# heitorrapela/HalluciDet

Measured on AMD Instinct MI355X. Metric: images/sec train_hallucidet (640x512, batch 8/GPU), higher is better.
Workload: dtype f16; 1 GPU; train_hallucidet.py fasterrcnn LLVIP batch=8 fp16 on 1xMI355X (BASELINE configs[1]); U-Net resnet34 fwd+bwd, 3 frozen Faster R-CNN R50-FPN passes @300x300 (one batched evaluation of 24 images: trunk, RPN, RoI heads, NMS for all three; the RGB / IR passes' LOSS VALUES, which the reference computes and discards, are not evaluated), loss scaling, value clip 0.5, Adam; global_batch=8, image=1x512x640 IR + 3x512x640 RGB, batch_per_gpu=8, parallelism=dp1

## Files before the change

### hallucidet_amd/_abi.py

```python
import ctypes as C
import os

_HERE = os.path.dirname(os.path.abspath(__file__))
LIB_PATH = os.environ.get("HD_HIP_LIB") or os.path.join(_HERE, "lib", "libhallucidet_hip.so")

ABI_VERSION = 6

HD_ACT_NONE, HD_ACT_RELU, HD_ACT_SIGMOID = 0, 1, 2
HD_OUT_NHWC_F16, HD_OUT_NCHW_F32, HD_OUT_NHWC_F32 = 0, 1, 2

c_i32 = C.c_int32
c_i64 = C.c_int64
c_f = C.c_float
c_d = C.c_double
vp = C.c_void_p


class HipLibraryMissing(RuntimeError):
    pass


class HipCallError(RuntimeError):
    pass

# ... 5 lines not shown
        ("C1", c_i32), ("C2", c_i32), ("Ho", c_i32), ("Wo", c_i32), ("Cout", c_i32),
        ("KH", c_i32), ("KW", c_i32), ("stride", c_i32), ("pad", c_i32),
        ("up1", c_i32), ("in_dil", c_i32), ("act", c_i32), ("out_mode", c_i32),
        ("in_scale", vp), ("in_shift", vp), ("in_relu", c_i32), ("out_pool2", c_i32),
        ("bs_y", vp), ("bs_z", vp), ("bs_mean", vp), ("bs_invstd", vp), ("bs_gamma", vp), ("bs_beta", vp), ("bs_relu", c_i32), ("reserved1", c_i32),
        ("y2", vp),
    ]


class WprepDesc(C.Structure):
    _fields_ = [("w_oihw", C.c_void_p), ("w_fwd", C.c_void_p), ("w_dgrad", C.c_void_p)] + \
               [(n, C.c_int32) for n in ("Cout", "Cin", "KH", "KW", "Cin_pad", "Cout_pad")]


class WredDesc(C.Structure):
    _fields_ = [("slab", C.c_void_p), ("dw_oihw", C.c_void_p)] + \
               [(n, C.c_int32) for n in ("nsplit", "Cout_slab", "Cout", "KH", "KW", "Cin", "Cin_real", "accumulate")] + \
               [("scale", C.c_float)] + [(n, C.c_int32) for n in ("mode", "first_block", "reserved")]


class WgradArgs(C.Structure):
    _fields_ = [
        ("x", vp), ("x2", vp), ("dy", vp), ("slab", vp),
        ("N", c_i32), ("Hsrc", c_i32), ("Wsrc", c_i32), ("Hin", c_i32), ("Win", c_i32),
        ("C1", c_i32), ("C2", c_i32), ("Ho", c_i32), ("Wo", c_i32), ("Cout", c_i32),
        ("KH", c_i32), ("KW", c_i32), ("stride", c_i32), ("pad", c_i32), ("up1", c_i32),
        ("nsplit", c_i32),
        ("in_scale", vp), ("in_shift", vp), ("in_relu", c_i32), ("reserved0", c_i32),
        ("dw_oihw", vp), ("dw_scale", c_f), ("reserved1", c_i32),
    ]


class ThinDgradArgs(C.Structure):
    _fields_ = [("ga", vp), ("gb", vp), ("wda", vp), ("wdb", vp), ("mask", vp), ("dx", vp), ("stride_a", c_i64), ("stride_b", c_i64)] + \
               [(n, c_i32) for n in ("n", "hw", "C", "Ka", "Kb", "Ka_p", "Kb_p", "g_f16")]


PROTOTYPES = {
    "hd_abi_version": (C.c_int, []),
    "hd_last_error": (C.c_char_p, []),
    "hd_arch": (C.c_char_p, []),
    "hd_conv2d": (C.c_int, [C.POINTER(ConvArgs), vp]),
    "hd_conv2d_stats_rows": (C.c_int, [C.POINTER(ConvArgs)]),
    "hd_conv2d_pool2_ok": (C.c_int, [C.POINTER(ConvArgs)]),
    "hd_conv2d_bstat_ok": (C.c_int, [C.POINTER(ConvArgs)]),
    "hd_conv2d_route": (C.c_int, [C.POINTER(ConvArgs), C.POINTER(c_i32)]),
    "hd_conv7x7s2_dgrad_thin": (C.c_int, [vp, vp, vp, vp] + [C.c_int] * 5 + [vp]),
    "hd_conv_tune_override": (C.c_int, [C.c_int] * 4),
    "hd_conv_tune_w8": (C.c_int, [C.c_int, C.c_int]),
    "hd_conv_nominal_batch": (C.c_int, [C.c_int]),
    "hd_gemm_w8_mode": (C.c_int, [C.c_int]),
    "hd_thin_gemm_mode": (C.c_int, [C.c_int]),
    "hd_thin_gemm_on": (C.c_int, []),
    "hd_thin_dgrad_pair": (C.c_int, [C.POINTER(ThinDgradArgs), vp]),
    "hd_thin_dgrad_pair_multi": (C.c_int, [C.POINTER(ThinDgradArgs), C.c_int, vp]),
    "hd_wgrad_w8_blocks": (C.c_int, [C.POINTER(WgradArgs)]),
    "hd_wgrad_route": (C.c_int, [C.POINTER(WgradArgs), C.POINTER(c_i32)]),
    "hd_wgrad": (C.c_int, [C.POINTER(WgradArgs), vp]),
    "hd_wgrad_multi": (C.c_int, [C.POINTER(WgradArgs), C.c_int, vp]),
    "hd_wgrad_direct_ok": (C.c_int, [C.POINTER(WgradArgs)]),
    "hd_conv2d_wgrad": (C.c_int, [C.POINTER(ConvArgs), C.POINTER(WgradArgs), vp]),
    "hd_conv2d_multi": (C.c_int, [C.POINTER(ConvArgs), C.c_int, vp]),
    "hd_wgrad_tune_override": (C.c_int, [C.c_int]),
    "hd_wgrad_reduce": (C.c_int, [vp, vp] + [C.c_int] * 7 + [c_f, C.c_int, vp]),
    "hd_wgrad_reduce_plan": (C.c_int, [vp, C.c_int]),
    "hd_wgrad_reduce_multi": (C.c_int, [vp, C.c_int, C.c_int, vp]),
    "hd_weight_prep": (C.c_int, [vp, vp, vp, vp] + [C.c_int] * 6 + [vp]),
    "hd_weight_prep_multi": (C.c_int, [vp, C.c_int, C.c_int, vp]),
    "hd_colsum": (C.c_int, [vp, C.c_int, C.c_int, vp, vp, vp]),
    "hd_rowsum": (C.c_int, [vp, C.c_int, C.c_int, vp, C.c_int, vp]),
    "hd_bn_finalize": (C.c_int, [vp, C.c_int, C.c_int, c_d, vp, vp, vp, vp, c_f, c_f, vp, vp, vp, vp, vp]),
    "hd_bn_eval_scale_shift": (C.c_int, [vp, vp, vp, vp, c_f, C.c_int, vp, vp, vp]),
    "hd_bn_apply": (C.c_int, [vp, vp, vp, vp, vp, c_i64, C.c_int, C.c_int, vp]),
    "hd_bn_bwd_reduce": (C.c_int, [vp] * 8 + [C.c_int, c_i64, C.c_int, C.c_int, vp]),
    "hd_bn_bwd_apply": (C.c_int, [vp] * 8 + [C.c_int] + [vp] * 5 + [c_f, C.c_int, c_i64, C.c_int, C.c_int, vp]),
    "hd_maxpool3x3s2": (C.c_int, [vp, vp] + [C.c_int] * 6 + [vp]),
    "hd_maxpool3x3s2_bwd": (C.c_int, [vp, vp, vp] + [C.c_int] * 6 + [vp]),
    "hd_maxpool3x3s2_idx": (C.c_int, [vp, vp, vp] + [C.c_int] * 6 + [vp]),
    "hd_maxpool3x3s2_bwd_idx": (C.c_int, [vp, vp, vp] + [C.c_int] * 6 + [vp]),
    "hd_maxpool3x3s2_bwd_idx_add": (C.c_int, [vp, vp, vp, vp] + [C.c_int] * 6 + [vp]),
    "hd_concat_up_bwd": (C.c_int, [vp, vp, vp] + [C.c_int] * 5 + [vp]),
    "hd_subsample2": (C.c_int, [vp, vp] + [C.c_int] * 6 + [vp]),
    "hd_subsample2_bwd": (C.c_int, [vp, vp] + [C.c_int] * 7 + [vp]),
    "hd_nchw_to_nhwc_resize": (C.c_int, [vp, vp] + [C.c_int] * 7 + [vp]),
    "hd_nchw_to_nhwc_resize_strided": (C.c_int, [vp, c_i64, c_i64, vp] + [C.c_int] * 7 + [vp]),
    "hd_nchw_to_nhwc_resize_bwd": (C.c_int, [vp, vp] + [C.c_int] * 7 + [c_f, vp]),
    "hd_image_resample": (C.c_int, [vp, c_i64, c_i64, vp] + [C.c_int] * 7 + [vp, vp, vp, C.c_int] * 2 + [vp, vp, vp, vp, vp]),
    "hd_image_resample_bwd": (C.c_int, [vp, vp] + [C.c_int] * 7 + [vp, vp, vp, C.c_int] * 2 + [vp, c_f, vp]),
    "hd_resample_taps_check": (C.c_int, [vp, vp, vp] + [C.c_int] * 3 + [vp, vp, vp, C.c_int, vp]),
    "hd_nhwc_to_nchw": (C.c_int, [vp, vp] + [C.c_int] * 5 + [vp]),
    "hd_upsample_add": (C.c_int, [vp, vp, vp] + [C.c_int] * 6 + [vp]),
    "hd_upsample_add_bwd": (C.c_int, [vp, vp] + [C.c_int] * 7 + [vp]),
    "hd_upsample2_bwd": (C.c_int, [vp, vp] + [C.c_int] * 7 + [vp]),
    "hd_add_f16": (C.c_int, [vp, vp, vp, c_i64, vp]),
    "hd_slice_channels": (C.c_int, [vp, vp, c_i64, C.c_int, C.c_int, C.c_int, C.c_int, vp]),
    "hd_sigmoid_bwd_nchw_to_nhwc": (C.c_int, [vp, vp, vp] + [C.c_int] * 5 + [c_f, vp]),
    "hd_relu_bwd": (C.c_int, [vp, vp, vp, c_i64, vp]),
    "hd_f32_to_f16": (C.c_int, [vp, vp, c_i64, c_f, vp]),
    "hd_f16_to_f32": (C.c_int, [vp, vp, c_i64, c_f, vp]),
    "hd_pad_cast_f32_f16": (C.c_int, [vp, vp, C.c_int64, C.c_int, C.c_int, C.c_int64, C.c_int64, vp]),
    "hd_pad_cast_f32_f16_multi": (C.c_int, [vp, vp, vp, vp, vp, vp, vp, C.c_int, vp]),
    "hd_channel_sum_f16": (C.c_int, [vp, c_i64, C.c_int, vp, C.c_int, vp]),
    "hd_scale_store": (C.c_int, [vp, vp, C.c_int, c_f, C.c_int, vp]),
    "hd_nms_sorted_batched": (C.c_int, [vp, vp, C.c_int, C.c_int, c_f, vp, vp, vp]),
    "hd_nms_sorted_batched_topk": (C.c_int, [vp, vp, C.c_int, C.c_int, c_f, vp, vp, C.c_int, vp]),
    "hd_roi_align": (C.c_int, [vp, vp, vp] + [C.c_int] * 7 + [c_f, C.c_int, vp]),
# ... 107 lines not shown
```

### hallucidet_amd/csrc/conv3x3_small.hip

```cpp
#include "hd_common.h"
#include "conv_params.h"

namespace {

typedef float f32x4_t __attribute__((ext_vector_type(4)));

constexpr int TH = 8, TW = 32;
constexpr int PH = TH + 2, PW = TW + 2;

__device__ __forceinline__ float row16_sum(float v) {
  v += __builtin_bit_cast(float, __builtin_amdgcn_update_dpp(0, __builtin_bit_cast(int, v), 0xB1, 0xF, 0xF, true));
  v += __builtin_bit_cast(float, __builtin_amdgcn_update_dpp(0, __builtin_bit_cast(int, v), 0x4E, 0xF, 0xF, true));
  v += __builtin_bit_cast(float, __builtin_amdgcn_update_dpp(0, __builtin_bit_cast(int, v), 0x141, 0xF, 0xF, true));
  v += __builtin_bit_cast(float, __builtin_amdgcn_update_dpp(0, __builtin_bit_cast(int, v), 0x140, 0xF, 0xF, true));
  return v;
}

template <int CIN, int COUT>
__global__ __launch_bounds__(256) void conv3x3_small_kernel(ConvP p) {
  constexpr int KTOT = 9 * CIN;
  constexpr int KSTEPS = (KTOT + 31) / 32;
  constexpr int KPAD = KSTEPS * 32;
  constexpr int MT = COUT / 16;
  constexpr int TPS = 32 / CIN;
  constexpr int PATCH_HALVES = PH * PW * CIN > 16 * TH * TW * 2 ? PH * PW * CIN : 16 * TH * TW * 2;
  __shared__ __attribute__((aligned(16))) f16 s_patch[PATCH_HALVES];
  __shared__ __attribute__((aligned(16))) f16 s_w[COUT * KPAD];
  __shared__ float s_red[4][COUT][2];

  const int tid = threadIdx.x, lane = tid & 63, wave = tid >> 6;
  const int tiles_x = (p.Wo + TW - 1) / TW, tiles_y = (p.Ho + TH - 1) / TH;
  const int tiles_total = p.N * tiles_x * tiles_y;

  for (int e = tid; e < COUT * KPAD / 8; e += 256) {
    const int co = e / (KPAD / 8), k8 = (e - co * (KPAD / 8)) * 8;
    f16x8 v = {0, 0, 0, 0, 0, 0, 0, 0};
    if (k8 < KTOT && co < p.Cout) v = *reinterpret_cast<const f16x8*>(p.w + (size_t)co * KTOT + k8);
    *reinterpret_cast<f16x8*>(s_w + co * KPAD + k8) = v;
  }
  constexpr int C8 = CIN / 8;
  constexpr int XL = (PH * PW * C8 + 255) / 256;
  f16x8 rx[XL];
  const bool fuse_bn = p.in_scale != nullptr;
  float isc[8], ish[8];
  if (fuse_bn) {
    const f32x4_t a0 = *reinterpret_cast<const f32x4_t*>(p.in_scale + (tid % C8) * 8), a1 = *reinterpret_cast<const f32x4_t*>(p.in_scale + (tid % C8) * 8 + 4);
    const f32x4_t b0 = *reinterpret_cast<const f32x4_t*>(p.in_shift + (tid % C8) * 8), b1 = *reinterpret_cast<const f32x4_t*>(p.in_shift + (tid % C8) * 8 + 4);
#pragma unroll
    for (int k = 0; k < 4; ++k) {
      isc[k] = a0[k]; isc[4 + k] = a1[k];
      ish[k] = b0[k]; ish[4 + k] = b1[k];
    }
  }
  const bool in_relu = p.in_relu != 0;
  unsigned vmask = 0;
  auto gload = [&](int tile) {
    vmask = 0;
    const bool live = tile < tiles_total;
    int b = live ? tile : 0;
    const int tx = b % tiles_x;
    b /= tiles_x;
    const int ty = b % tiles_y;
    const int n = b / tiles_y;
    const f16* xb = p.x + (size_t)n * p.Hsrc * p.Wsrc * CIN;
#pragma unroll
    for (int i = 0; i < XL; ++i) {
      const int e = tid + i * 256;
      const int c8 = e % C8, pp = e / C8;
// ... 36 lines not shown
    __syncthreads();
    gload(tile + gridDim.x);

    f32x4_t acc[4][MT];
#pragma unroll
    for (int t = 0; t < 4; ++t)
#pragma unroll
      for (int m = 0; m < MT; ++m) acc[t][m] = (f32x4_t){0.f, 0.f, 0.f, 0.f};
#pragma unroll
    for (int ks = 0; ks < KSTEPS; ++ks) {
      int tap = ks * TPS + (g * 8) / CIN;
      const int ci0 = (g * 8) % CIN;
      if (tap > 8) tap = 8;
      const int kh = tap / 3, kw = tap - kh * 3;
      f16x8 af[MT];
#pragma unroll
      for (int m = 0; m < MT; ++m) af[m] = *reinterpret_cast<const f16x8*>(s_w + (m * 16 + pl) * KPAD + ks * 32 + g * 8);
#pragma unroll
      for (int t = 0; t < 4; ++t) {
        const int oy = wave * 2 + (t >> 1), ox = (t & 1) * 16 + pl;
        const f16x8 bf = *reinterpret_cast<const f16x8*>(s_patch + ((oy + kh) * PW + ox + kw) * CIN + ci0);
#pragma unroll
        for (int m = 0; m < MT; ++m) acc[t][m] = __builtin_amdgcn_mfma_f32_16x16x32_f16(af[m], bf, acc[t][m], 0, 0, 0);
      }
    }

    if (p.out_mode == HD_OUT_NCHW_F32) {
      float* yf = reinterpret_cast<float*>(p.y) + (size_t)n * p.Cout * p.Ho * p.Wo;
      float* s_out = reinterpret_cast<float*>(s_patch);
      __syncthreads();
#pragma unroll
      for (int t = 0; t < 4; ++t) {
        const int oyl = wave * 2 + (t >> 1), oxl = (t & 1) * 16 + pl;
#pragma unroll
        for (int r = 0; r < 4; ++r) {
          const int co = g * 4 + r;
          if (co < p.Cout) {
            float v = acc[t][0][r] + (p.bias ? p.bias[co] : 0.f);
            if (p.act == HD_ACT_RELU) v = fmaxf(v, 0.f);
            else if (p.act == HD_ACT_SIGMOID) v = 1.f / (1.f + __expf(-v));
            s_out[(co * TH + oyl) * TW + oxl] = v;
          }
        }
      }
      __syncthreads();
      {
        const int oyl = tid / TW, oxl = tid - oyl * TW;
        if (y0 + oyl < p.Ho && x0 + oxl < p.Wo)
          for (int co = 0; co < p.Cout; ++co) yf[((size_t)co * p.Ho + y0 + oyl) * p.Wo + x0 + oxl] = s_out[(co * TH + oyl) * TW + oxl];
      }
      continue;
    }
    if (p.pool2) {
      f16* yb2 = reinterpret_cast<f16*>(p.y) + (size_t)n * (p.Ho >> 1) * (p.Wo >> 1) * COUT;
#pragma unroll
      for (int t = 0; t < 2; ++t) {
        const int oy = y0 + wave * 2, ox = x0 + t * 16 + pl;
#pragma unroll
        for (int m = 0; m < MT; ++m) {
          f16x4 o;
#pragma unroll
          for (int r = 0; r < 4; ++r) {
            float v = acc[t][m][r] + acc[t + 2][m][r];
            v += __builtin_bit_cast(float, __builtin_amdgcn_update_dpp(0, __builtin_bit_cast(int, v), 0xB1, 0xF, 0xF, true));
            o[r] = (f16)v;
          }
          if (!(pl & 1) && oy < p.Ho && ox < p.Wo)
            *reinterpret_cast<f16x4*>(yb2 + ((size_t)(oy >> 1) * (p.Wo >> 1) + (ox >> 1)) * COUT + m * 16 + g * 4) = o;
        }
      }
      continue;
    }
    f16* yb = reinterpret_cast<f16*>(p.y) + (size_t)n * p.Ho * p.Wo * COUT;
    float ssum[MT][4], ssq[MT][4];
#pragma unroll
    for (int m = 0; m < MT; ++m)
#pragma unroll
      for (int r = 0; r < 4; ++r) ssum[m][r] = ssq[m][r] = 0.f;
#pragma unroll
    for (int t = 0; t < 4; ++t) {
      const int oy = y0 + wave * 2 + (t >> 1), ox = x0 + (t & 1) * 16 + pl;
      if (oy < p.Ho && ox < p.Wo) {
#pragma unroll
        for (int m = 0; m < MT; ++m) {
          f16x4 o;
#pragma unroll
          for (int r = 0; r < 4; ++r) {
            o[r] = (f16)acc[t][m][r];
            const float vr = (float)o[r];
            ssum[m][r] += vr;
            ssq[m][r] += vr * vr;
          }
          *reinterpret_cast<f16x4*>(yb + ((size_t)oy * p.Wo + ox) * COUT + m * 16 + g * 4) = o;
        }
      }
    }
    if (p.stats) {
#pragma unroll
      for (int m = 0; m < MT; ++m)
#pragma unroll
        for (int r = 0; r < 4; ++r) {
          ssum[m][r] = row16_sum(ssum[m][r]);
          ssq[m][r] = row16_sum(ssq[m][r]);
        }
      if (pl == 0) {
#pragma unroll
        for (int m = 0; m < MT; ++m)
#pragma unroll
          for (int r = 0; r < 4; ++r) {
            s_red[wave][m * 16 + g * 4 + r][0] = ssum[m][r];
            s_red[wave][m * 16 + g * 4 + r][1] = ssq[m][r];
          }
      }
      __syncthreads();
      if (tid < COUT) {
        float s = 0.f, s2 = 0.f;
#pragma unroll
        for (int w4 = 0; w4 < 4; ++w4) {
          s += s_red[w4][tid][0];
          s2 += s_red[w4][tid][1];
        }
        p.stats[((size_t)tile * 2 + 0) * COUT + tid] = s;
        p.stats[((size_t)tile * 2 + 1) * COUT + tid] = s2;
      }
    }
  }
}

}

bool hd_conv_small_eligible(const ConvP& p) {
  if (!(p.KH == 3 && p.KW == 3 && p.stride == 1 && p.pad == 1 && p.in_dil == 1 && p.C2 == 0 && p.x2 == nullptr &&
        (p.C1 == 8 || p.C1 == 16 || p.C1 == 32) && !p.res && !p.mask && p.Ho == p.Hin && p.Wo == p.Win))
    return false;
  if (p.out_mode == HD_OUT_NHWC_F32) return false;
  if (p.out_mode == HD_OUT_NCHW_F32) return p.Cout <= 16 && !p.stats;
  return (p.Cout == 16 || p.Cout == 32) && !p.bias && p.act == HD_ACT_NONE;
}

bool hd_conv_small_pool2_ok(const ConvP& p) {
  return hd_conv_small_eligible(p) && p.out_mode == HD_OUT_NHWC_F16 && !p.stats && !p.in_scale && (p.Ho % 2) == 0 && (p.Wo % 2) == 0 &&
         (p.pool2 == 0 || (p.pool2 == p.Cout && !p.y2));
}

int hd_conv_small_tiles(const ConvP& p) { return p.N * hd_cdiv(p.Ho, TH) * hd_cdiv(p.Wo, TW); }

void hd_conv_launch_small(ConvP& p, hipStream_t s) {
  const int tiles = hd_conv_small_tiles(p);
  dim3 grid(tiles < 1536 ? tiles : 1536);
#define LAUNCH(CI, CO) hipLaunchKernelGGL((conv3x3_small_kernel<CI, CO>), grid, dim3(256), 0, s, p)
  if (p.C1 == 8) { if (p.Cout <= 16) LAUNCH(8, 16); else LAUNCH(8, 32); }
  else if (p.C1 == 16) { if (p.Cout <= 16) LAUNCH(16, 16); else LAUNCH(16, 32); }
  else { if (p.Cout <= 16) LAUNCH(32, 16); else LAUNCH(32, 32); }
#undef LAUNCH
}
```

### hallucidet_amd/csrc/conv_dispatch.hip

```cpp
#include <stdlib.h>

#include "conv_params.h"

namespace {

int pick_bn(int Cout) { return Cout > 64 ? 128 : (Cout > 32 ? 64 : 32); }
int pick_bm(int M, int Cout) {
  int bn = pick_bn(Cout);
  int64_t blocks128 = (int64_t)hd_cdiv(M, 128) * hd_cdiv(Cout, bn);
  return (bn > 32 && blocks128 < 512) ? 64 : 128;
}

int fill_params(const hd_conv_args* a, ConvP& p) {
  HD_CHECK_ARG(a && a->x && a->w && a->y, "hd_conv2d: null pointer");
  HD_CHECK_ARG(a->C1 > 0 && a->C1 % 8 == 0 && a->C2 >= 0 && a->C2 % 8 == 0, "hd_conv2d: channel counts must be multiples of 8 (C1=%d C2=%d)", a->C1, a->C2);
  HD_CHECK_ARG((a->C2 == 0) == (a->x2 == nullptr), "hd_conv2d: x2/C2 mismatch");
  HD_CHECK_ARG(a->N > 0 && a->Ho > 0 && a->Wo > 0 && a->Cout > 0 && a->KH > 0 && a->KW > 0 && a->stride > 0, "hd_conv2d: bad extent");
  HD_CHECK_ARG(!(a->in_dil > 1 && (a->up1 || a->C2)), "hd_conv2d: in_dil excludes up1/x2");
  HD_CHECK_ARG(a->in_dil <= 2, "hd_conv2d: in_dil must be 1 or 2 (strides on the hot path)");
  HD_CHECK_ARG(a->C2 == 0 || (a->C1 % 32 == 0 && a->C2 % 32 == 0), "hd_conv2d: dual-source gather needs C1, C2 multiples of 32 (a K tile holds channels of one source)");
  HD_CHECK_ARG(!a->up1 || (a->Hin == 2 * a->Hsrc && a->Win == 2 * a->Wsrc), "hd_conv2d: up1 needs Hin=2*Hsrc");
  HD_CHECK_ARG((int64_t)a->N * a->Ho * a->Wo < (1ll << 31), "hd_conv2d: too many pixels");
  p.x = (const f16*)a->x;
  p.x2 = (const f16*)a->x2;
// ... 4 lines not shown
  p.y = a->y;
  p.stats = a->stats;
  p.N = a->N; p.Hsrc = a->Hsrc; p.Wsrc = a->Wsrc; p.Hin = a->Hin; p.Win = a->Win;
  p.C1 = a->C1; p.C2 = a->C2; p.Cin = a->C1 + a->C2;
  p.Ho = a->Ho; p.Wo = a->Wo; p.Cout = a->Cout; p.KH = a->KH; p.KW = a->KW;
  p.stride = a->stride; p.pad = a->pad; p.up1 = a->up1; p.in_dil = a->in_dil < 1 ? 1 : a->in_dil;
  p.act = a->act; p.out_mode = a->out_mode;
  HD_CHECK_ARG((a->in_scale == nullptr) == (a->in_shift == nullptr), "hd_conv2d: in_scale / in_shift must be given together");
  p.in_scale = a->in_scale; p.in_shift = a->in_shift; p.in_relu = a->in_relu;
  p.pool2 = a->out_pool2;
  p.y2 = a->y2;
  p.bs_y = (const f16*)a->bs_y; p.bs_z = (const f16*)a->bs_z;
  p.bs_mean = a->bs_mean; p.bs_invstd = a->bs_invstd; p.bs_gamma = a->bs_gamma; p.bs_beta = a->bs_beta; p.bs_relu = a->bs_relu;
  HD_CHECK_ARG(!p.bs_y || (p.stats && p.bs_mean && p.bs_invstd && !a->mask && a->act == HD_ACT_NONE && a->out_mode == HD_OUT_NHWC_F16 && !a->bias),
               "hd_conv2d: bs_* (BatchNorm backward sums) need stats, bs_mean, bs_invstd and exclude mask / act / bias / non-f16 output");
  HD_CHECK_ARG(p.out_mode >= HD_OUT_NHWC_F16 && p.out_mode <= HD_OUT_NHWC_F32, "hd_conv2d: out_mode %d", p.out_mode);
  p.M = a->N * a->Ho * a->Wo;
  p.cin8 = p.Cin / 8;
  p.nchunks = a->KH * a->KW * p.cin8;
  p.nk = 0;
  p.Ktot = a->KH * a->KW * p.Cin;
  p.prio = 0;
  p.par = p.ph = p.pw = p.Hc = p.Wc = p.t0h = p.t0w = 0;
  p.gm = p.gn = 0;
  p.tgroup = 1;
  p.inv_cin8 = 1.0f / (float)p.cin8;
  p.inv_kw = 1.0f / (float)a->KW;
  int64_t xb = (int64_t)a->N * a->Hsrc * a->Wsrc * a->C1 * 2;
  int64_t x2b = a->x2 ? (int64_t)a->N * a->Hin * a->Win * a->C2 * 2 : 0;
  int64_t wb = (int64_t)a->Cout * p.Ktot * 2;
  HD_CHECK_ARG(xb < 0xFFFFFFF0ll && x2b < 0xFFFFFFF0ll && wb < 0xFFFFFFF0ll, "hd_conv2d: tensor larger than 4 GiB (buffer addressing)");
  p.xbytes = (unsigned)xb; p.x2bytes = (unsigned)x2b; p.wbytes = (unsigned)wb;
#ifdef HD_CONV_TRACE
  p.trace = nullptr;
  p.trace_tid = 0;
#endif
  return HD_OK;
}

int env_int(const char* name, int dflt) {
  const char* v = getenv(name);
  return v ? atoi(v) : dflt;
}

}

static bool g_small_ok = true;

bool use_small(const ConvP& p) {
  static const int on = env_int("HD_CONV_SMALL", 1);
  return on && g_small_ok && hd_conv_small_eligible(p);
}

bool use_c64(const ConvP& p) {
  static const int on = env_int("HD_CONV_C64", 1);
  return on && g_small_ok && hd_conv_c64_eligible(p);
}

bool use_stem(const ConvP& p) {
  static const int on = env_int("HD_CONV_STEM", 1);
  return on && g_small_ok && hd_conv_stem_eligible(p);
}

bool use_c32(const ConvP& p) {
  static const int on = env_int("HD_CONV_C32", 1);
  return on && g_small_ok && !p.stats && hd_conv_c32to128_eligible(p);
}

bool use_cat(const ConvP& p) {
  static const int on = env_int("HD_CONV_CAT", 1);
  return on && g_small_ok && hd_conv_cat128to32_eligible(p);
}

static int g_gemm8_mode = -1;
extern "C" int hd_gemm_w8_mode(int mode) {
  HD_CHECK_ARG(mode == -1 || mode == 0 || mode == 128 || mode == 1128, "hd_gemm_w8_mode: mode in {-1, 0, 128, 1128}");
  g_gemm8_mode = mode;
  return HD_OK;
}
bool hd_gemm_w8_eligible(const ConvP& p);
void hd_gemm_w8_launch(ConvP& p, int tile, hipStream_t s);
static int choose_gemm8(const ConvP& p) {
  static const int on = env_int("HD_GEMM8", 1);
  if (!on || g_gemm8_mode == 0 || !g_small_ok || !hd_gemm_w8_eligible(p)) return 0;
  if (g_gemm8_mode > 0) return g_gemm8_mode;
  if (p.res || p.M < 2048 || p.Cout < 512 || p.Ktot < 512) return 0;
  const int64_t t128 = (int64_t)hd_cdiv(p.M, 256) * hd_cdiv(p.Cout, 128), t1128 = (int64_t)hd_cdiv(p.M, 128) * hd_cdiv(p.Cout, 128);
  if (t128 >= 160 && t128 <= 256) return 128;
  if (t1128 >= 200) return 1128;
  return 0;
}

static int g_thin_mode = -1;
static bool thin_on() {
  static const int on = env_int("HD_THIN_GEMM", 1);
  return on && g_thin_mode != 0;
}
extern "C" int hd_thin_gemm_mode(int mode) {
  HD_CHECK_ARG(mode == -1 || mode == 0 || mode == 1, "hd_thin_gemm_mode: mode in {-1, 0, 1}");
  g_thin_mode = mode;
  return HD_OK;
}
extern "C" int hd_thin_gemm_on(void) { return thin_on() ? 1 : 0; }
bool hd_thin_fwd_eligible(const ConvP& p);
int hd_thin_fwd_rg(int64_t rows);
void hd_thin_fwd_launch(const ConvP* ps, int n, hipStream_t s);
// ... 379 lines not shown
```

### hallucidet_amd/csrc/conv_params.h

```cpp
#pragma once
#include <stdlib.h>

#include "hd_common.h"

struct ConvP {
  const f16* x;
  const f16* x2;
  const f16* w;
  const float* bias;
  const f16* res;
  const f16* mask;
  void* y;
  void* y2;
  float* stats;
  unsigned xbytes, x2bytes, wbytes;
  int N, Hsrc, Wsrc, Hin, Win, C1, C2, Cin, Ho, Wo, Cout, KH, KW, stride, pad, up1, in_dil, act, out_mode;
  int M, cin8, nchunks, nk, Ktot;
  int gm, gn;
  int tgroup;
  float inv_cin8, inv_kw;
  int par, ph, pw, Hc, Wc, t0h, t0w;
  int pool2;
  int prio;
  const float* in_scale;
// ... 63 lines not shown
  const int rem = m - n * hw;
  const int i = fast ? hd_fdiv(rem, p.Wc, hd_rcp(p.Wc)) : rem / p.Wc;
  const int jj = rem - i * p.Wc;
  return (n * p.Ho + 2 * i + p.ph) * p.Wo + 2 * jj + p.pw;
}

static inline int hd_conv_tile_order(const ConvP& p) {
  static const int on = [] { const char* v = getenv("HD_CONV_TGROUP"); return v ? atoi(v) : 1; }();
  const double A = (double)p.xbytes + (double)p.x2bytes, W = (double)p.wbytes;
  if (!on || p.par || p.gm < 2 || p.gn < 2 || W <= 4.0e6) return 1;
  int best_s = 1;
  double best = 1e30;
  for (int s = 1; s <= 8; s *= 2) {
    if (s > 1 && A * s / 8.0 > 2.0e6) break;
    const double t = s * A + 8.0 * W / s;
    if (t < best) { best = t; best_s = s; }
  }
  const int g = (p.gm * best_s + 7) / 8;
  return g < 1 ? 1 : g;
}
__device__ __forceinline__ void hd_conv_tile_of(const ConvP& p, int bid, int& tile_m, int& tile_n) {
  if (p.tgroup <= 1) {
    tile_m = bid / p.gn;
    tile_n = bid - tile_m * p.gn;
  } else {
    const int width = p.tgroup * p.gn;
    const int gid = bid / width;
    const int first_m = gid * p.tgroup;
    const int gsz = p.gm - first_m < p.tgroup ? p.gm - first_m : p.tgroup;
    const int r = bid - gid * width;
    tile_n = r / gsz;
    tile_m = first_m + r - tile_n * gsz;
  }
}

void hd_conv_launch_bk32(ConvP& p, int bm, int bn, bool deep, hipStream_t s);
void hd_conv_launch_bk64(ConvP& p, int bm, int bn, bool deep, hipStream_t s);
bool hd_conv_launch_bk32_multi(ConvMulti& mp, int bm, int bn, bool deep, hipStream_t s);
bool hd_conv_launch_bk64_multi(ConvMulti& mp, int bm, int bn, bool deep, hipStream_t s);
bool hd_conv_p8_eligible(const ConvP& p);
bool hd_conv_p8_pool2_ok(const ConvP& p);
int hd_conv_p8_tiles(const ConvP& p, int cfg);
void hd_conv_launch_p8(ConvP& p, int cfg, hipStream_t s);
bool hd_conv_m160_eligible(const ConvP& p);
bool hd_conv_m160_pool2_ok(const ConvP& p);
int hd_conv_m160_tiles(const ConvP& p, int th, int tw);
void hd_conv_launch_m160(ConvP& p, int th, int tw, hipStream_t s);
void hd_conv_launch_m96_multi(ConvMulti& mp, hipStream_t s);
void hd_conv_launch_p8_wgrad(ConvP& p, int cfg, const hd_wgrad_args* wa, hipStream_t s);
bool hd_conv_small_eligible(const ConvP& p);
bool hd_conv_small_pool2_ok(const ConvP& p);
int hd_conv_small_tiles(const ConvP& p);
void hd_conv_launch_small(ConvP& p, hipStream_t s);
bool hd_conv_c64_eligible(const ConvP& p);
int hd_conv_c64_rows(const ConvP& p);
bool hd_conv_c32to128_eligible(const ConvP& p);
void hd_conv_launch_c32to128(ConvP& p, hipStream_t s);
bool hd_conv_cat128to32_eligible(const ConvP& p);
int hd_conv_cat128to32_rows(const ConvP& p);
void hd_conv_launch_cat128to32(ConvP& p, hipStream_t s);
bool hd_conv_stem_eligible(const ConvP& p);
int hd_conv_stem_rows(const ConvP& p);
void hd_conv_launch_stem(ConvP& p, hipStream_t s);
void hd_conv_launch_c64(ConvP& p, hipStream_t s);
```

### hallucidet_amd/ops.py

```python
import collections
import ctypes as C
import os
import threading

import numpy as np
import torch

from . import _abi
from . import resample as _resample
from ._abi import ConvArgs, WgradArgs, check, ptr
from .resample import resample_taps

ACT_NONE, ACT_RELU, ACT_SIGMOID = 0, 1, 2

_tls = threading.local()


def act_dtype():
    return getattr(_tls, "dtype", torch.float16)


class storage:
    def __init__(self, dtype):
        assert dtype in (torch.float16, torch.float32)
# ... 435 lines not shown
    check(_abi.fn("hd_groupnorm8_relu_bwd", x)(ptr(dy), ptr(x), ptr(y), ptr(gamma), ptr(stat), ptr(dx), N, H * W, C_, 1 if relu else 0, _stream()),
          "hd_groupnorm8_relu_bwd")
    return dx


def groupnorm8_param_grad(dy, x, y, stat, dgamma, dbeta, scale=1.0, *, relu=True, accumulate=True):
    _need_cuda(dy, x, stat, dgamma, dbeta)
    N, H, W, C_ = x.shape
    check(_abi.fn("hd_groupnorm8_param_grad", x)(ptr(dy), ptr(x), ptr(y), ptr(stat), ptr(dgamma), ptr(dbeta), N, H * W, C_, 1 if relu else 0,
                                               float(scale), 1 if accumulate else 0, _stream()), "hd_groupnorm8_param_grad")


def pad_cast_f32_f16(x, cp, dtype=None):
    _need_cuda(x)
    n, H, W, C_ = x.shape
    assert x.stride()[1:] == (W * C_, C_, 1) or n * H * W == 0
    y = torch.empty((n, H, W, cp), dtype=dtype or act_dtype(), device=x.device)
    img_stride = x.stride(0) if n > 1 else H * W * C_
    check(_abi.fn("hd_pad_cast_f32_f16", y)(ptr(x), ptr(y), n * H * W, C_, cp, H * W, max(img_stride, H * W * C_), _stream()), "hd_pad_cast_f32_f16")
    return y


def pad_cast_f32_f16_many(xs, cps, dtype=None):
    if len(xs) == 1:
        return [pad_cast_f32_f16(xs[0], cps[0], dtype=dtype)]
    _need_cuda(*xs)
    outs = []
    for lo in range(0, len(xs), 16):
        part = xs[lo:lo + 16]
        n = len(part)
        ys, Ps, Cs, Cps, rpis, strides = [], [], [], [], [], []
        for x, cp in zip(part, cps[lo:lo + 16]):
            b, H, W, C_ = x.shape
            assert x.dtype == torch.float32 and (x.stride()[1:] == (W * C_, C_, 1) or b * H * W == 0)
            y = torch.empty((b, H, W, cp), dtype=dtype or act_dtype(), device=x.device)
            ys.append(y); Ps.append(b * H * W); Cs.append(C_); Cps.append(cp); rpis.append(max(H * W, 1))
            strides.append(max(x.stride(0) if b > 1 else H * W * C_, H * W * C_))
        arr = lambda ctype, vals: (ctype * n)(*vals)
        check(_abi.fn("hd_pad_cast_f32_f16_multi", ys[0])(arr(C.c_void_p, [x.data_ptr() for x in part]), arr(C.c_void_p, [y.data_ptr() for y in ys]),
                                                          arr(C.c_int64, Ps), arr(C.c_int, Cs), arr(C.c_int, Cps), arr(C.c_int64, rpis),
                                                          arr(C.c_int64, strides), n, _stream()), "hd_pad_cast_f32_f16_multi")
        outs += ys
    return outs


def thin_gemm_mode(mode):
    check(_abi.load().hd_thin_gemm_mode(int(mode)), "hd_thin_gemm_mode")


def thin_gemm_on():
    return _abi.load().hd_thin_gemm_on() == 1


THIN_MULTI_MAX = 8


def thin_dgrad_pair_many(calls):
    assert 1 <= len(calls) <= THIN_MULTI_MAX
    args, outs = [], []
    for ga, gb, wda, wdb, mask in calls:
        _need_cuda(ga, gb, wda, wdb, mask)
        n, H, W, Ka = ga.shape
        Kb = gb.shape[3]
        C_, Kap = wda.shape
        Kbp = wdb.shape[1]
        assert gb.shape[:3] == ga.shape[:3] and wdb.shape[0] == C_ and wda.dtype == wdb.dtype == torch.float16 and wda.is_contiguous() and wdb.is_contiguous()
        f16 = ga.dtype == torch.float16
        assert gb.dtype == ga.dtype and ga.dtype in (torch.float16, torch.float32)
        if f16:
            assert ga.is_contiguous() and gb.is_contiguous() and Ka == Kap and Kb == Kbp
            sa = sb = 0
        else:
            assert ga.stride()[1:] == (W * Ka, Ka, 1) and gb.stride()[1:] == (W * Kb, Kb, 1)
            sa = max(ga.stride(0) if n > 1 else 0, H * W * Ka)
            sb = max(gb.stride(0) if n > 1 else 0, H * W * Kb)
        assert mask is None or (mask.shape == (n, H, W, C_) and mask.dtype == torch.float16 and mask.is_contiguous())
        dx = torch.empty((n, H, W, C_), dtype=torch.float16, device=ga.device)
        args.append(_abi.ThinDgradArgs(ptr(ga), ptr(gb), ptr(wda), ptr(wdb), ptr(mask), ptr(dx), sa, sb, n, H * W, C_, Ka, Kb, Kap, Kbp, 1 if f16 else 0))
        outs.append(dx)
    arr = (_abi.ThinDgradArgs * len(args))(*args)
    check(_abi.load().hd_thin_dgrad_pair_multi(arr, len(args), _stream()), "hd_thin_dgrad_pair_multi")
    return outs


def maxpool3x3s2(x):
    N, H, W, C_ = x.shape
    Ho, Wo = (H - 1) // 2 + 1, (W - 1) // 2 + 1
    y = torch.empty((N, Ho, Wo, C_), dtype=x.dtype, device=x.device)
    check(_abi.fn("hd_maxpool3x3s2", x)(ptr(x), ptr(y), N, H, W, C_, Ho, Wo, _stream()), "hd_maxpool3x3s2")
    return y


def maxpool3x3s2_idx(x):
    N, H, W, C_ = x.shape
    Ho, Wo = (H - 1) // 2 + 1, (W - 1) // 2 + 1
    y = torch.empty((N, Ho, Wo, C_), dtype=x.dtype, device=x.device)
    idx = torch.empty((N, Ho, Wo, C_), dtype=torch.uint8, device=x.device)
    check(_abi.fn("hd_maxpool3x3s2_idx", x)(ptr(x), ptr(y), ptr(idx), N, H, W, C_, Ho, Wo, _stream()), "hd_maxpool3x3s2_idx")
    return y, idx


def maxpool3x3s2_bwd_idx(idx, dy, in_hw, add=None):
    N, Ho, Wo, C_ = dy.shape
    H, W = in_hw
    dx = torch.empty((N, H, W, C_), dtype=dy.dtype, device=dy.device)
    if add is None:
# ... 905 lines not shown
```

### include/hallucidet_hip.h

```cpp
#ifndef HALLUCIDET_HIP_H
#define HALLUCIDET_HIP_H

#include <stdint.h>

#ifdef __cplusplus
extern "C" {
#endif

#define HD_OK 0
#define HD_E_ARG (-1)
#define HD_E_LAUNCH (-2)
#define HD_E_UNSUPPORTED (-3)

#define HD_ACT_NONE 0
#define HD_ACT_RELU 1
#define HD_ACT_SIGMOID 2

#define HD_OUT_NHWC_F16 0
#define HD_OUT_NCHW_F32 1
#define HD_OUT_NHWC_F32 2

int hd_abi_version(void);
const char* hd_last_error(void);
const char* hd_arch(void);

typedef struct hd_conv_args {
  const void* x;
  const void* x2;
  const void* w;
  const float* bias;
  const void* res;
  const void* mask;
  void* y;
  float* stats;
  int32_t N, Hsrc, Wsrc;
  int32_t Hin, Win;
  int32_t C1, C2;
  int32_t Ho, Wo, Cout;
  int32_t KH, KW, stride, pad;
  int32_t up1, in_dil;
  int32_t act, out_mode;
  const float* in_scale;
  const float* in_shift;
  int32_t in_relu;
  int32_t out_pool2;
  const void* bs_y;
  const void* bs_z;
  const float* bs_mean;
  const float* bs_invstd;
  const float* bs_gamma;
  const float* bs_beta;
  int32_t bs_relu, reserved1;
  void* y2;
} hd_conv_args;

int hd_conv2d(const hd_conv_args* a, void* stream);
int hd_conv2d_bstat_ok(const hd_conv_args* a);
int hd_conv2d_pool2_ok(const hd_conv_args* a);
int hd_conv2d_stats_rows(const hd_conv_args* a);
int hd_conv2d_route(const hd_conv_args* a, int32_t out[8]);
int hd_conv7x7s2_dgrad_thin(const void* dy, const void* mask_z, const void* w16, void* dx, int N, int Hl, int Wl, int H, int W, void* stream);
int hd_conv_tune_override(int bm, int bn, int bk, int deep);
int hd_conv_tune_w8(int cfg, int nslices);
int hd_conv_nominal_batch(int n);
int hd_gemm_w8_mode(int mode);
int hd_thin_gemm_mode(int mode);
int hd_thin_gemm_on(void);

typedef struct hd_thin_dgrad_args {
  const void* ga;
  const void* gb;
  const void* wda;
  const void* wdb;
  const void* mask;
  void* dx;
  int64_t stride_a, stride_b;
  int32_t n, hw, C, Ka, Kb, Ka_p, Kb_p, g_f16;
} hd_thin_dgrad_args;
int hd_thin_dgrad_pair(const hd_thin_dgrad_args* a, void* stream);
#define HD_THIN_MULTI_MAX 8
int hd_thin_dgrad_pair_multi(const hd_thin_dgrad_args* args, int n, void* stream);

typedef struct hd_wgrad_args {
  const void* x;
  const void* x2;
  const void* dy;
  float* slab;
  int32_t N, Hsrc, Wsrc, Hin, Win, C1, C2, Ho, Wo, Cout;
  int32_t KH, KW, stride, pad, up1;
  int32_t nsplit;
  const float* in_scale;
  const float* in_shift;
  int32_t in_relu, reserved0;
  float* dw_oihw;
  float dw_scale;
  int32_t reserved1;
} hd_wgrad_args;
int hd_wgrad(const hd_wgrad_args* a, void* stream);
int hd_wgrad_direct_ok(const hd_wgrad_args* a);
#define HD_WGRAD_MULTI_MAX 24
int hd_wgrad_multi(const hd_wgrad_args* args, int n, void* stream);
int hd_wgrad_w8_blocks(const hd_wgrad_args* a);
int hd_wgrad_route(const hd_wgrad_args* a, int32_t out[8]);
int hd_wgrad_tune_override(int tm);
int hd_conv2d_multi(const hd_conv_args* args, int n, void* stream);

int hd_conv2d_wgrad(const hd_conv_args* dgrad, const hd_wgrad_args* wgrad, void* stream);

int hd_wgrad_reduce(const float* slab, float* dw_oihw, int nsplit, int Cout_slab, int Cout, int KH, int KW,
                    int Cin, int Cin_real, float scale, int accumulate, void* stream);

#define HD_WRED_MAX 16
typedef struct hd_wred_desc {
  const float* slab;
  float* dw_oihw;
  int32_t nsplit, Cout_slab, Cout, KH, KW, Cin, Cin_real, accumulate;
  float scale;
  int32_t mode, first_block, reserved;
} hd_wred_desc;
int hd_wgrad_reduce_plan(hd_wred_desc* table_host, int n);
// ... 273 lines not shown
```

Before: 861.4 images/s.

## Add double-buffered persistent v2 kernel for small-channel 3x3 convolutions

Result: no change. 865.6 images/s, median of 6 (+0.5%).

```diff
diff --git a/hallucidet_amd/_abi.py b/hallucidet_amd/_abi.py
--- a/hallucidet_amd/_abi.py
+++ b/hallucidet_amd/_abi.py
@@ -81,6 +81,7 @@
     "hd_gemm_w8_mode": (C.c_int, [C.c_int]),
     "hd_thin_gemm_mode": (C.c_int, [C.c_int]),
     "hd_thin_gemm_on": (C.c_int, []),
+    "hd_small_conv_mode": (C.c_int, [C.c_int]),
     "hd_thin_dgrad_pair": (C.c_int, [C.POINTER(ThinDgradArgs), vp]),
     "hd_thin_dgrad_pair_multi": (C.c_int, [C.POINTER(ThinDgradArgs), C.c_int, vp]),
     "hd_wgrad_w8_blocks": (C.c_int, [C.POINTER(WgradArgs)]),
diff --git a/hallucidet_amd/csrc/conv3x3_small.hip b/hallucidet_amd/csrc/conv3x3_small.hip
--- a/hallucidet_amd/csrc/conv3x3_small.hip
+++ b/hallucidet_amd/csrc/conv3x3_small.hip
@@ -1,9 +1,13 @@
+#include <type_traits>
+
 #include "hd_common.h"
 #include "conv_params.h"
+#include "hd_lds_dma.h"
 
 namespace {
 
 typedef float f32x4_t __attribute__((ext_vector_type(4)));
+typedef uint32_t u32x2 __attribute__((ext_vector_type(2)));
 
 constexpr int TH = 8, TW = 32;
 constexpr int PH = TH + 2, PW = TW + 2;
@@ -14,6 +18,67 @@
   v += __builtin_bit_cast(float, __builtin_amdgcn_update_dpp(0, __builtin_bit_cast(int, v), 0x141, 0xF, 0xF, true));
   v += __builtin_bit_cast(float, __builtin_amdgcn_update_dpp(0, __builtin_bit_cast(int, v), 0x140, 0xF, 0xF, true));
   return v;
+}
+
+template <int COUT, bool BUF>
+__device__ __forceinline__ void store_pool2(const ConvP& p, const f32x4_t (&acc)[4][COUT / 16], int n, int y0, int x0, int wave, int pl, int g) {
+  constexpr int MT = COUT / 16;
+  f16* yb2 = reinterpret_cast<f16*>(p.y) + (size_t)n * (p.Ho >> 1) * (p.Wo >> 1) * COUT;
+  const __amdgpu_buffer_rsrc_t ry = __builtin_amdgcn_make_buffer_rsrc(yb2, 0, BUF ? (unsigned)(p.Ho >> 1) * (p.Wo >> 1) * COUT * 2 : 0, 0x00020000);
+#pragma unroll
+  for (int t = 0; t < 2; ++t) {
+    const int oy = y0 + wave * 2, ox = x0 + t * 16 + pl;
+#pragma unroll
+    for (int m = 0; m < MT; ++m) {
+      f16x4 o;
+#pragma unroll
+      for (int r = 0; r < 4; ++r) {
+        float v = acc[t][m][r] + acc[t + 2][m][r];
+        v += __builtin_bit_cast(float, __builtin_amdgcn_update_dpp(0, __builtin_bit_cast(int, v), 0xB1, 0xF, 0xF, true));
+        o[r] = (f16)v;
+      }
+      const bool inb = !(pl & 1) && oy < p.Ho && ox < p.Wo;
+      if (BUF)
+        __builtin_amdgcn_raw_buffer_store_b64(__builtin_bit_cast(u32x2, o), ry,
+                                              inb ? (((unsigned)(oy >> 1) * (p.Wo >> 1) + (ox >> 1)) * COUT + m * 16 + g * 4) * 2 : OOB, 0, 0);
+      else if (inb)
+        *reinterpret_cast<f16x4*>(yb2 + ((size_t)(oy >> 1) * (p.Wo >> 1) + (ox >> 1)) * COUT + m * 16 + g * 4) = o;
+    }
+  }
+}
+
+template <int COUT, bool BUF>
+__device__ __forceinline__ void store_plain(const ConvP& p, const f32x4_t (&acc)[4][COUT / 16], int n, int y0, int x0, int wave, int pl, int g,
+                                            float (&ssum)[COUT / 16][4], float (&ssq)[COUT / 16][4]) {
+  constexpr int MT = COUT / 16;
+  f16* yb = reinterpret_cast<f16*>(p.y) + (size_t)n * p.Ho * p.Wo * COUT;
+  const __amdgpu_buffer_rsrc_t ry = __builtin_amdgcn_make_buffer_rsrc(yb, 0, BUF ? (unsigned)p.Ho * p.Wo * COUT * 2 : 0, 0x00020000);
+#pragma unroll
+  for (int m = 0; m < MT; ++m)
+#pragma unroll
+    for (int r = 0; r < 4; ++r) ssum[m][r] = ssq[m][r] = 0.f;
+#pragma unroll
+  for (int t = 0; t < 4; ++t) {
+    const int oy = y0 + wave * 2 + (t >> 1), ox = x0 + (t & 1) * 16 + pl;
+    const bool inb = oy < p.Ho && ox < p.Wo;
+#pragma unroll
+    for (int m = 0; m < MT; ++m) {
+      f16x4 o;
+#pragma unroll
+      for (int r = 0; r < 4; ++r) {
+        o[r] = (f16)acc[t][m][r];
+        const float vr = (float)o[r];
+        if (inb) {
+          ssum[m][r] += vr;
+          ssq[m][r] += vr * vr;
+        }
+      }
+      if (BUF)
+        __builtin_amdgcn_raw_buffer_store_b64(__builtin_bit_cast(u32x2, o), ry, inb ? (((unsigned)oy * p.Wo + ox) * COUT + m * 16 + g * 4) * 2 : OOB, 0, 0);
+      else if (inb)
+        *reinterpret_cast<f16x4*>(yb + ((size_t)oy * p.Wo + ox) * COUT + m * 16 + g * 4) = o;
+    }
+  }
 }
 
 template <int CIN, int COUT>
@@ -156,49 +221,11 @@
       continue;
     }
     if (p.pool2) {
-      f16* yb2 = reinterpret_cast<f16*>(p.y) + (size_t)n * (p.Ho >> 1) * (p.Wo >> 1) * COUT;
-#pragma unroll
-      for (int t = 0; t < 2; ++t) {
-        const int oy = y0 + wave * 2, ox = x0 + t * 16 + pl;
-#pragma unroll
-        for (int m = 0; m < MT; ++m) {
-          f16x4 o;
-#pragma unroll
-          for (int r = 0; r < 4; ++r) {
-            float v = acc[t][m][r] + acc[t + 2][m][r];
-            v += __builtin_bit_cast(float, __builtin_amdgcn_update_dpp(0, __builtin_bit_cast(int, v), 0xB1, 0xF, 0xF, true));
-            o[r] = (f16)v;
-          }
-          if (!(pl & 1) && oy < p.Ho && ox < p.Wo)
-            *reinterpret_cast<f16x4*>(yb2 + ((size_t)(oy >> 1) * (p.Wo >> 1) + (ox >> 1)) * COUT + m * 16 + g * 4) = o;
-        }
-      }
+      store_pool2<COUT, false>(p, acc, n, y0, x0, wave, pl, g);
       continue;
     }
-    f16* yb = reinterpret_cast<f16*>(p.y) + (size_t)n * p.Ho * p.Wo * COUT;
     float ssum[MT][4], ssq[MT][4];
-#pragma unroll
-    for (int m = 0; m < MT; ++m)
-#pragma unroll
-      for (int r = 0; r < 4; ++r) ssum[m][r] = ssq[m][r] = 0.f;
-#pragma unroll
-    for (int t = 0; t < 4; ++t) {
-      const int oy = y0 + wave * 2 + (t >> 1), ox = x0 + (t & 1) * 16 + pl;
-      if (oy < p.Ho && ox < p.Wo) {
-#pragma unroll
-        for (int m = 0; m < MT; ++m) {
-          f16x4 o;
-#pragma unroll
-          for (int r = 0; r < 4; ++r) {
-            o[r] = (f16)acc[t][m][r];
-            const float vr = (float)o[r];
-            ssum[m][r] += vr;
-            ssq[m][r] += vr * vr;
-          }
-          *reinterpret_cast<f16x4*>(yb + ((size_t)oy * p.Wo + ox) * COUT + m * 16 + g * 4) = o;
-        }
-      }
-    }
+    store_plain<COUT, false>(p, acc, n, y0, x0, wave, pl, g, ssum, ssq);
     if (p.stats) {
 #pragma unroll
       for (int m = 0; m < MT; ++m)
@@ -228,6 +255,247 @@
         p.stats[((size_t)tile * 2 + 1) * COUT + tid] = s2;
       }
     }
+  }
+}
+
+
+constexpr int small_blocks_per_cu(int cin, int cout) { return cin * cout <= 128 ? 4 : cin * cout <= 256 ? 3 : 2; }
+
+template <int CIN, int COUT, bool UP>
+__global__ __launch_bounds__(256) __attribute__((amdgpu_waves_per_eu(small_blocks_per_cu(CIN, COUT)))) void conv3x3_small_kernel_v2(ConvP p) {
+  constexpr int KTOT = 9 * CIN;
+  constexpr int KSTEPS = (KTOT + 31) / 32;
+  constexpr int MT = COUT / 16;
+  constexpr int TPS = 32 / CIN;
+  constexpr int SPH = UP ? TH / 2 + 2 : PH, SPW = UP ? TW / 2 + 2 : PW;
+  constexpr int PITCH = (UP && CIN == 32) ? 56 : CIN;
+  constexpr int C8 = CIN / 8;
+  constexpr int NVEC = SPH * SPW * C8;
+  constexpr int XL = (NVEC + 255) / 256;
+  __shared__ __attribute__((aligned(16))) f16 s_patch[2][SPH * SPW * PITCH];
+  __shared__ float s_red[2][4][COUT][2];
+  constexpr bool WREG = KSTEPS * MT < 18;
+  constexpr int WP = ((KSTEPS * 4 + 13) / 16 * 16 + 2) * 8;
+  __shared__ __attribute__((aligned(16))) f16 s_w[WREG ? 8 : COUT * WP];
+
+  constexpr int RES = 256 * small_blocks_per_cu(CIN, COUT);
+  const int stride = (int)gridDim.x < RES ? (int)gridDim.x : RES;
+  if ((int)blockIdx.x >= stride) return;
+  const int tid = threadIdx.x, lane = tid & 63, wave = tid >> 6;
+  const int pl = lane & 15, g = lane >> 4;
+  const int tiles_x = (p.Wo + TW - 1) / TW, tiles_y = (p.Ho + TH - 1) / TH;
+  const int tiles_total = p.N * tiles_x * tiles_y;
+  const float inv_tx = hd_rcp(tiles_x), inv_ty = hd_rcp(tiles_y);
+  const int HB = UP ? p.Hsrc : p.Hin, WB = UP ? p.Wsrc : p.Win;
+
+  f16x8 af[WREG ? KSTEPS : 1][MT];
+  if (WREG) {
+#pragma unroll
+    for (int ks = 0; ks < (WREG ? KSTEPS : 1); ++ks)
+#pragma unroll
+      for (int m = 0; m < MT; ++m) {
+        const int co = m * 16 + pl, k8 = ks * 32 + g * 8;
+        f16x8 v = {0, 0, 0, 0, 0, 0, 0, 0};
+        if (k8 < KTOT && co < p.Cout) v = *reinterpret_cast<const f16x8*>(p.w + (size_t)co * KTOT + k8);
+        af[ks][m] = v;
+      }
+  } else {
+    for (int e = tid; e < COUT * KSTEPS * 4; e += 256) {
+      const int co = e / (KSTEPS * 4), k8 = (e - co * (KSTEPS * 4)) * 8;
+      f16x8 v = {0, 0, 0, 0, 0, 0, 0, 0};
+      if (k8 < KTOT && co < p.Cout) v = *reinterpret_cast<const f16x8*>(p.w + (size_t)co * KTOT + k8);
+      *reinterpret_cast<f16x8*>(s_w + co * WP + k8) = v;
+    }
+  }
+
+  int pyx[XL], lds_off[XL];
+  unsigned relb[XL];
+#pragma unroll
+  for (int i = 0; i < XL; ++i) {
+    const int e = tid + i * 256;
+    const int c8 = e % C8, pp = e / C8;
+    const int py = pp / SPW, px = pp - py * SPW;
+    pyx[i] = py | (px << 8);
+    lds_off[i] = PITCH == CIN ? e * 8 : pp * PITCH + c8 * 8;
+    relb[i] = (unsigned)(((py * WB + px) * CIN + c8 * 8) * 2);
+  }
+  const bool fuse_bn = p.in_scale != nullptr;
+  float isc[8], ish[8];
+  if (fuse_bn) {
+    const f32x4_t a0 = *reinterpret_cast<const f32x4_t*>(p.in_scale + (tid % C8) * 8), a1 = *reinterpret_cast<const f32x4_t*>(p.in_scale + (tid % C8) * 8 + 4);
+    const f32x4_t b0 = *reinterpret_cast<const f32x4_t*>(p.in_shift + (tid % C8) * 8), b1 = *reinterpret_cast<const f32x4_t*>(p.in_shift + (tid % C8) * 8 + 4);
+#pragma unroll
+    for (int k = 0; k < 4; ++k) {
+      isc[k] = a0[k]; isc[4 + k] = a1[k];
+      ish[k] = b0[k]; ish[4 + k] = b1[k];
+    }
+  }
+  const bool in_relu = p.in_relu != 0;
+  const bool head = p.out_mode == HD_OUT_NCHW_F32;
+  float hbias[4] = {0.f, 0.f, 0.f, 0.f};
+  if (head && p.bias) {
+#pragma unroll
+    for (int r = 0; r < 4; ++r)
+      if (g * 4 + r < p.Cout) hbias[r] = p.bias[g * 4 + r];
+  }
+
+  auto boff = [&](int ks, int t) -> int {
+    int tap = ks * TPS + (g * 8) / CIN;
+    const int ci0 = (g * 8) % CIN;
+    if (tap > 8) tap = 8;
+    const int kh = tap / 3, kw = tap - kh * 3;
+    if (UP) return ((wave + (((t >> 1) + kh + 1) >> 1)) * SPW + (t & 1) * 8 + ((pl + kw + 1) >> 1)) * PITCH + ci0;
+    return ((wave * 2 + (t >> 1) + kh) * SPW + (t & 1) * 16 + pl + kw) * PITCH + ci0;
+  };
+
+  const __amdgpu_buffer_rsrc_t rx = __builtin_amdgcn_make_buffer_rsrc(const_cast<f16*>(p.x), 0, p.xbytes, 0x00020000);
+  const __amdgpu_buffer_rsrc_t rst = __builtin_amdgcn_make_buffer_rsrc(p.stats, 0, p.stats ? (unsigned)tiles_total * 2 * COUT * 4 : 0, 0x00020000);
+  u32x4 rxv[2][XL];
+  unsigned vm[2] = {0, 0};
+  int tn[2] = {0, 0}, ty0[2] = {0, 0}, tx0[2] = {0, 0};
+  auto gload = [&](auto P, int tile) __attribute__((always_inline)) {
+    constexpr int q = decltype(P)::value;
+    const bool live = tile < tiles_total;
+    const int b = live ? tile : 0;
+    const int qq = hd_fdiv(b, tiles_x, inv_tx);
+    const int tx = b - qq * tiles_x;
+    const int n = hd_fdiv(qq, tiles_y, inv_ty);
+    const int ty = qq - n * tiles_y;
+    tn[q] = n; ty0[q] = ty * TH; tx0[q] = tx * TW;
+    const int Y0 = UP ? (ty * TH >> 1) - 1 : ty * TH - 1, X0 = UP ? (tx * TW >> 1) - 1 : tx * TW - 1;
+    const unsigned base = (unsigned)(((((int64_t)n * HB + Y0) * WB + X0) * CIN) * 2);
+    unsigned m = 0;
+#pragma unroll
+    for (int i = 0; i < XL; ++i) {
+      const int hy = Y0 + (pyx[i] & 255), wx = X0 + (pyx[i] >> 8);
+      const bool ok = live && tid + i * 256 < NVEC && (unsigned)hy < (unsigned)HB && (unsigned)wx < (unsigned)WB;
+      rxv[q][i] = __builtin_amdgcn_raw_buffer_load_b128(rx, ok ? base + relb[i] : OOB, 0, 0);
+      m |= ok ? 1u << i : 0u;
+    }
+    vm[q] = m;
+  };
+
+  int prev_tile = -1, prev_par = 0;
+  auto fold_stats = [&](int b, int tile) __attribute__((always_inline)) {
+    float s = 0.f, s2 = 0.f;
+    const int c = tid < COUT ? tid : 0;
+#pragma unroll
+    for (int w4 = 0; w4 < 4; ++w4) {
+      s += s_red[b][w4][c][0];
+      s2 += s_red[b][w4][c][1];
+    }
+    const unsigned o = tid < COUT ? (unsigned)(((size_t)tile * 2 * COUT + tid) * 4) : OOB;
+    __builtin_amdgcn_raw_buffer_store_b32(__builtin_bit_cast(unsigned, s), rst, o, 0, 0);
+    __builtin_amdgcn_raw_buffer_store_b32(__builtin_bit_cast(unsigned, s2), rst, tid < COUT ? o + COUT * 4 : OOB, 0, 0);
+  };
+
+  auto step = [&](auto P, int tile) __attribute__((always_inline)) {
+    constexpr int q = decltype(P)::value;
+    const int n = tn[q], y0 = ty0[q], x0 = tx0[q];
+    f16* sp = s_patch[q];
+#pragma unroll
+    for (int i = 0; i < XL; ++i) {
+      f16x8 v = __builtin_bit_cast(f16x8, rxv[q][i]);
+      if (fuse_bn) {
+        f16x8 z;
+#pragma unroll
+        for (int k = 0; k < 8; ++k) {
+          float f = hd_bn_affine((float)v[k], isc[k], ish[k]);
+          if (in_relu) f = fmaxf(f, 0.f);
+          z[k] = (f16)f;
+        }
+        const bool real = (vm[q] >> i) & 1u;
+        const u32x4 zz = __builtin_bit_cast(u32x4, z);
+#pragma unroll
+        for (int k = 0; k < 4; ++k) rxv[q][i][k] = real ? zz[k] : rxv[q][i][k];
+        v = __builtin_bit_cast(f16x8, rxv[q][i]);
+      }
+      if (tid + i * 256 < NVEC) *reinterpret_cast<f16x8*>(sp + lds_off[i]) = v;
+    }
+    __syncthreads();
+    if (p.stats && prev_tile >= 0) fold_stats(q ^ 1, prev_tile);
+    gload(P, tile + 2 * stride);
+
+    f32x4_t acc[4][MT];
+#pragma unroll
+    for (int t = 0; t < 4; ++t)
+#pragma unroll
+      for (int m = 0; m < MT; ++m) acc[t][m] = (f32x4_t){0.f, 0.f, 0.f, 0.f};
+#pragma unroll
+    for (int ks = 0; ks < KSTEPS; ++ks) {
+      f16x8 a[MT];
+#pragma unroll
+      for (int m = 0; m < MT; ++m) a[m] = WREG ? af[WREG ? ks : 0][m] : *reinterpret_cast<const f16x8*>(s_w + (m * 16 + pl) * WP + ks * 32 + g * 8);
+#pragma unroll
+      for (int t = 0; t < 4; ++t) {
+        const f16x8 bf = *reinterpret_cast<const f16x8*>(sp + boff(ks, t));
+#pragma unroll
+        for (int m = 0; m < MT; ++m) acc[t][m] = __builtin_amdgcn_mfma_f32_16x16x32_f16(a[m], bf, acc[t][m], 0, 0, 0);
+      }
+    }
+    prev_tile = tile;
+    prev_par = q;
+
+    if (head) {
+      const size_t img = (size_t)p.Cout * p.Ho * p.Wo * 4;
+      const __amdgpu_buffer_rsrc_t ry = __builtin_amdgcn_make_buffer_rsrc(reinterpret_cast<char*>(p.y) + (size_t)n * img, 0, (unsigned)img, 0x00020000);
+#pragma unroll
+      for (int t = 0; t < 4; ++t) {
+        const int oy = y0 + wave * 2 + (t >> 1), ox = x0 + (t & 1) * 16 + pl;
+        const bool inb = oy < p.Ho && ox < p.Wo;
+#pragma unroll
+        for (int r = 0; r < 4; ++r) {
+          const int co = g * 4 + r;
+          float v = acc[t][0][r] + hbias[r];
+          if (p.act == HD_ACT_RELU) v = fmaxf(v, 0.f);
+          else if (p.act == HD_ACT_SIGMOID) v = 1.f / (1.f + __expf(-v));
+          __builtin_amdgcn_raw_buffer_store_b32(__builtin_bit_cast(unsigned, v), ry, inb && co < p.Cout ? (((unsigned)co * p.Ho + oy) * p.Wo + ox) * 4 : OOB, 0, 0);
+        }
+      }
+      return;
+    }
+    if (p.pool2) {
+      store_pool2<COUT, true>(p, acc, n, y0, x0, wave, pl, g);
+      return;
+    }
+    float ssum[MT][4], ssq[MT][4];
+    store_plain<COUT, true>(p, acc, n, y0, x0, wave, pl, g, ssum, ssq);
+    if (p.stats) {
+#pragma unroll
+      for (int m = 0; m < MT; ++m)
+#pragma unroll
+        for (int r = 0; r < 4; ++r) {
+          ssum[m][r] = row16_sum(ssum[m][r]);
+          ssq[m][r] = row16_sum(ssq[m][r]);
+        }
+      if (pl == 0) {
+#pragma unroll
+        for (int m = 0; m < MT; ++m)
+#pragma unroll
+          for (int r = 0; r < 4; ++r) {
+            s_red[q][wave][m * 16 + g * 4 + r][0] = ssum[m][r];
+            s_red[q][wave][m * 16 + g * 4 + r][1] = ssq[m][r];
+          }
+      }
+    }
+  };
+
+  const std::integral_constant<int, 0> c0;
+  const std::integral_constant<int, 1> c1;
+  int tile = blockIdx.x;
+  gload(c0, tile);
+  gload(c1, tile + stride);
+  for (;;) {
+    if (tile >= tiles_total) break;
+    step(c0, tile);
+    tile += stride;
+    if (tile >= tiles_total) break;
+    step(c1, tile);
+    tile += stride;
+  }
+  if (p.stats && prev_tile >= 0) {
+    __syncthreads();
+    fold_stats(prev_par, prev_tile);
   }
 }
 
@@ -249,10 +517,18 @@
 
 int hd_conv_small_tiles(const ConvP& p) { return p.N * hd_cdiv(p.Ho, TH) * hd_cdiv(p.Wo, TW); }
 
+static bool small_v2(const ConvP& p) { return hd_small_conv_v2_on() && (int64_t)p.Ho * p.Wo * 64 < 0xFFFFFFF0ll; }
+
 void hd_conv_launch_small(ConvP& p, hipStream_t s) {
   const int tiles = hd_conv_small_tiles(p);
   dim3 grid(tiles < 1536 ? tiles : 1536);
-#define LAUNCH(CI, CO) hipLaunchKernelGGL((conv3x3_small_kernel<CI, CO>), grid, dim3(256), 0, s, p)
+  const bool v2 = small_v2(p);
+#define LAUNCH(CI, CO)                                                                                          \
+  do {                                                                                                          \
+    if (!v2) hipLaunchKernelGGL((conv3x3_small_kernel<CI, CO>), grid, dim3(256), 0, s, p);                      \
+    else if (p.up1) hipLaunchKernelGGL((conv3x3_small_kernel_v2<CI, CO, true>), grid, dim3(256), 0, s, p);      \
+    else hipLaunchKernelGGL((conv3x3_small_kernel_v2<CI, CO, false>), grid, dim3(256), 0, s, p);                \
+  } while (0)
   if (p.C1 == 8) { if (p.Cout <= 16) LAUNCH(8, 16); else LAUNCH(8, 32); }
   else if (p.C1 == 16) { if (p.Cout <= 16) LAUNCH(16, 16); else LAUNCH(16, 32); }
   else { if (p.Cout <= 16) LAUNCH(32, 16); else LAUNCH(32, 32); }
diff --git a/hallucidet_amd/csrc/conv_dispatch.hip b/hallucidet_amd/csrc/conv_dispatch.hip
--- a/hallucidet_amd/csrc/conv_dispatch.hip
+++ b/hallucidet_amd/csrc/conv_dispatch.hip
@@ -80,6 +80,17 @@
   return on && g_small_ok && hd_conv_small_eligible(p);
 }
 
+static int g_small_v2_mode = -1;
+bool hd_small_conv_v2_on() {
+  static const int on = env_int("HD_SMALL_CONV_V2", 1);
+  return on && g_small_v2_mode != 0;
+}
+extern "C" int hd_small_conv_mode(int mode) {
+  HD_CHECK_ARG(mode == -1 || mode == 0 || mode == 1, "hd_small_conv_mode: mode in {-1, 0, 1}");
+  g_small_v2_mode = mode;
+  return HD_OK;
+}
+
 bool use_c64(const ConvP& p) {
   static const int on = env_int("HD_CONV_C64", 1);
   return on && g_small_ok && hd_conv_c64_eligible(p);
diff --git a/hallucidet_amd/csrc/conv_params.h b/hallucidet_amd/csrc/conv_params.h
--- a/hallucidet_amd/csrc/conv_params.h
+++ b/hallucidet_amd/csrc/conv_params.h
@@ -139,6 +139,7 @@
 bool hd_conv_small_pool2_ok(const ConvP& p);
 int hd_conv_small_tiles(const ConvP& p);
 void hd_conv_launch_small(ConvP& p, hipStream_t s);
+bool hd_small_conv_v2_on();
 bool hd_conv_c64_eligible(const ConvP& p);
 int hd_conv_c64_rows(const ConvP& p);
 bool hd_conv_c32to128_eligible(const ConvP& p);
diff --git a/hallucidet_amd/ops.py b/hallucidet_amd/ops.py
--- a/hallucidet_amd/ops.py
+++ b/hallucidet_amd/ops.py
@@ -511,6 +511,10 @@
     return _abi.load().hd_thin_gemm_on() == 1
 
 
+def small_conv_mode(mode):
+    check(_abi.load().hd_small_conv_mode(int(mode)), "hd_small_conv_mode")
+
+
 THIN_MULTI_MAX = 8
 
 
diff --git a/include/hallucidet_hip.h b/include/hallucidet_hip.h
--- a/include/hallucidet_hip.h
+++ b/include/hallucidet_hip.h
@@ -66,6 +66,7 @@
 int hd_gemm_w8_mode(int mode);
 int hd_thin_gemm_mode(int mode);
 int hd_thin_gemm_on(void);
+int hd_small_conv_mode(int mode);
 
 typedef struct hd_thin_dgrad_args {
   const void* ga;
```
